# interactiveaudiolab/ppgs

Hardware: AMD Instinct MI355X
Metric: PPG frames/sec (whole node), mel repr, batch=32x1000 frames (higher is better)
Workload: dtype bf16; 1 GPU; configs[1]: mel representation, batch=32 x 1000 frames per GPU, audio resident in HBM -> (32,40,1000) fp32 posteriors in HBM; batch=32, frames=1000, per_gpu_batches=1, parallelism=utterance-sharded x1, no data-path collective

## Files before the change

### ppgs_amd/csrc/ppg_layer32.h

```cpp
#pragma once

#include "ppg_device.h"
#include "ppg_launch.h"

#include <type_traits>
#include <utility>

namespace {

constexpr float kLnEps32 = 1e-5f;
constexpr int HC = 128;

constexpr int tile_blocks(int hidt) { return hidt == 256 ? 5 : 3; }
template <int HIDT, int TBN_ = tile_blocks(HIDT)>
struct Geo {
    static_assert(HIDT == 256 || HIDT == 512, "hidden width");
    static constexpr int RB = HIDT / 128;
    static constexpr int KS = HIDT / 16;
    static constexpr int KH = KS / 16;
    static constexpr int TBN = TBN_;
    static constexpr int TOKS = 32 * TBN;
    static constexpr int HBUFS = TBN_ == tile_blocks(HIDT) ? 1 : 2;
    static constexpr int L_ACT = 0;
    static constexpr int L_H = TBN * KS * 1024;
    static constexpr int L_LNP1 = L_H + HBUFS * TBN * 8 * 1024;
    static constexpr int L_LNP2 = L_LNP1 + 3 * HIDT * 4;
    static constexpr int L_BQ = L_LNP2 + 3 * HIDT * 4;
    static constexpr int L_STATS = L_BQ + 3 * HIDT * 4;
    static constexpr int L_B1 = L_STATS + 2 * 4 * TOKS * 4;
};

__device__ __forceinline__ uint32_t lds_addr32(const void* p) {
    return (uint32_t)(uintptr_t)(const __attribute__((address_space(3))) void*)p;
}
template <int OFF>
__device__ __forceinline__ void ds_read128(u32x4& dst, uint32_t addr) {
    asm volatile("ds_read_b128 %0, %1 offset:%2" : "=v"(dst) : "v"(addr), "n"(OFF));
}
template <int N>
__device__ __forceinline__ void lgkm_wait32(u32x4& r) {
    asm volatile("s_waitcnt lgkmcnt(%1)" : "+v"(r) : "n"(N) : "memory");
    __builtin_amdgcn_sched_barrier(0);
}
template <int OFF>
__device__ __forceinline__ void gload128(u32x4& dst, uint32_t voff, const char* sbase) {
    asm volatile("global_load_dwordx4 %0, %1, %2 offset:%3" : "=v"(dst) : "v"(voff), "s"(sbase), "n"(OFF) : "memory");
}
template <int OFF>
__device__ __forceinline__ void gload128_acc(u32x4& dst, uint32_t voff, const char* sbase) {
    asm volatile("global_load_dwordx4 %0, %1, %2 offset:%3" : "=a"(dst) : "v"(voff), "s"(sbase), "n"(OFF) : "memory");
}
template <int K>
__device__ __forceinline__ void gload_frag(u32x4& dst, uint32_t voff, const char* base) {
    gload128<(K % 4) * 1024>(dst, voff, base + (K / 4) * 4096);
}
template <int K>
__device__ __forceinline__ void gload_frag_acc(u32x4& dst, uint32_t voff, const char* base) {
    gload128_acc<(K % 4) * 1024>(dst, voff, base + (K / 4) * 4096);
}
template <int COUNT>
__device__ __forceinline__ void vm_wait_all(u32x4 (&r)[COUNT]) {
    asm volatile("s_waitcnt vmcnt(0)" ::: "memory");
#pragma unroll
    for (int i = 0; i < COUNT; ++i) asm volatile("" : "+v"(r[i]));
    __builtin_amdgcn_sched_barrier(0);
}
__device__ __forceinline__ void glds16(const char* uniform_base, uint32_t lane_off, uint32_t lds_wave_addr) {
    const uint64_t b = reinterpret_cast<uint64_t>(uniform_base);
    const uint64_t base = ((uint64_t)(uint32_t)__builtin_amdgcn_readfirstlane((int)(b >> 32)) << 32) |
                          (uint64_t)(uint32_t)__builtin_amdgcn_readfirstlane((int)(uint32_t)b);
    asm volatile("s_mov_b32 m0, %2\n\ts_nop 0\n\tglobal_load_lds_dwordx4 %0, %1"
                 :: "v"(lane_off), "s"(base), "s"(__builtin_amdgcn_readfirstlane(lds_wave_addr)) : "memory", "m0");
}

template <class OFFS, int I, int N, int D, class USE>
__device__ __forceinline__ void stream_step(u32x4 (&ring)[D], uint32_t b0, uint32_t b1, USE& use) {
    if constexpr (I < N) {
        lgkm_wait32<(N - 1 - I < D - 1) ? (N - 1 - I) : (D - 1)>(ring[I % D]);
        use(std::integral_constant<int, I>{}, ring[I % D]);
        if constexpr (I + D < N) {
            constexpr int off = OFFS::at(I + D);
            if constexpr (off < 65536) ds_read128<off>(ring[I % D], b0); else ds_read128<off - 65536>(ring[I % D], b1);
        }
        stream_step<OFFS, I + 1, N, D>(ring, b0, b1, use);
    }
}
template <class OFFS, int I, int N, int D>
__device__ __forceinline__ void stream_prime(u32x4 (&ring)[D], uint32_t b0, uint32_t b1) {
    if constexpr (I < D && I < N) {
        constexpr int off = OFFS::at(I);
        if constexpr (off < 65536) ds_read128<off>(ring[I], b0); else ds_read128<off - 65536>(ring[I], b1);
        stream_prime<OFFS, I + 1, N, D>(ring, b0, b1);
    }
}
template <class OFFS, int N, int D, class USE>
__device__ __forceinline__ void stream(uint32_t b0, uint32_t b1, USE use) {
    u32x4 ring[D];
    stream_prime<OFFS, 0, N, D>(ring, b0, b1);
    stream_step<OFFS, 0, N, D>(ring, b0, b1, use);
}
template <int KS, int K0, int TB0, int NTB>
struct OffPanel { static constexpr int at(int i) { return ((TB0 + i % NTB) * KS + K0 + i / NTB) * 1024; } };
template <int TBN>
struct OffH { static constexpr int at(int i) { return ((i % TBN) * 8 + i / TBN) * 1024; } };

template <int TBN, int PAR>
struct OffH2 { static constexpr int at(int i) { return PAR * (TBN * 8 * 1024) + ((i % TBN) * 8 + i / TBN) * 1024; } };

struct OffChunk256 {
    static constexpr int at(int i) {
        constexpr int KS = Geo<256>::KS, HOFF = Geo<256>::L_H - Geo<256>::L_ACT;
        if (i < 48) return ((i % 3) * KS + i / 3) * 1024;
        if (i < 80) return ((3 + (i - 48) % 2) * KS + (i - 48) / 2) * 1024;
        if (i < 104) return HOFF + (((i - 80) % 3) * 8 + (i - 80) / 3) * 1024;
        return HOFF + ((3 + (i - 104) % 2) * 8 + (i - 104) / 2) * 1024;
    }
};

__device__ __forceinline__ void stat4(f32x2& sum2, f32x2& sq2, float v0, float v1, float v2, float v3) {
    const f32x2 a = {v0, v1}, b = {v2, v3};
    sum2 += a;
    sq2 = __builtin_elementwise_fma(a, a, sq2);
    sum2 += b;
    sq2 = __builtin_elementwise_fma(b, b, sq2);
}
__device__ __forceinline__ float hsum2(f32x2 v) {
    float r;
    asm("v_add_f32 %0, %1, %2" : "=v"(r) : "v"(v.x), "v"(v.y));
    return r;
}
__device__ __forceinline__ float pair_sum(float v) {
    auto b = __builtin_amdgcn_permlane32_swap(__float_as_uint(v), __float_as_uint(v), false, false);
    return __uint_as_float(b[0]) + __uint_as_float(b[1]);
}

template <class P, int HIDT, int TBS = tile_blocks(HIDT)>
__device__ __forceinline__ void panel_store(uint32_t pb0, int wave, int t, int rb, const f32x16& y) {
    using G = Geo<HIDT, TBS>;
#pragma unroll
    for (int s = 0; s < 2; ++s) {
        const u32x4 frag = u32x4{P::pack2(y[8 * s + 0], y[8 * s + 1]), P::pack2(y[8 * s + 2], y[8 * s + 3]),
                                 P::pack2(y[8 * s + 4], y[8 * s + 5]), P::pack2(y[8 * s + 6], y[8 * s + 7])};
        const uint32_t addr = pb0 + (uint32_t)((t * G::KS + 2 * G::RB * wave + 2 * rb + s) * 1024);
        asm volatile("ds_write_b128 %0, %1" :: "v"(addr), "v"(frag) : "memory");
    }
}

template <class P, int HIDT, int TBS = tile_blocks(HIDT)>
__device__ __forceinline__ void qkv_tail(const Layer32Args& a, char* smem, const int m0, u32x4 (&w1f)[16], u32x4 (&w2f)[16],
                                         const int nblk = TBS) {
    using G = Geo<HIDT, TBS>;
    constexpr int RB = G::RB, KS = G::KS, KH = G::KH, TB = G::TBN, TOKS = G::TOKS;
    constexpr int NSTEP = 3 * RB, NHS = NSTEP * KH;
    constexpr int NMMA = 16 * TB;
    constexpr int NU = 2 * TB;
    constexpr int USTRIDE = (NMMA - 16) / NU;
    const int lane = threadIdx.x & 63;
    const int wave = __builtin_amdgcn_readfirstlane(threadIdx.x >> 6);
    const int tok = lane & 31, hh = lane >> 5;
    const uint32_t voff = lane * 16;
    const uint32_t pb0 = lds_addr32(smem) + G::L_ACT + lane * 16, pb1 = pb0 + 65536;
    const int fbase = 32 * RB * wave;
    const f32x16 zero = {0.f, 0.f, 0.f, 0.f, 0.f, 0.f, 0.f, 0.f, 0.f, 0.f, 0.f, 0.f, 0.f, 0.f, 0.f, 0.f};
    asm volatile("s_waitcnt lgkmcnt(0)" ::: "memory");
    __syncthreads();
    const float* bq = reinterpret_cast<const float*>(smem + G::L_BQ);
    int vcol[TB][2];
    bool valigned[TB];
    bool regular = m0 + TOKS <= a.M && nblk == TB;
#pragma unroll
    for (int t = 0; t < TB; ++t) {
#pragma unroll
        for (int h = 0; h < 2; ++h) {
            const int mb = m0 + 32 * t + 16 * h;
            vcol[t][h] = -1;
            if (mb < a.M && t < nblk) {
                const int w = a.blk_win[mb >> 4];
                if (w >= 0) {
                    const int ttb = mb - a.win[w].tok_off;
                    vcol[t][h] = a.win[w].vt_off + (ttb >> 5) * 32 + 4 * ((ttb >> 4) & 1);
                }
            }
        }
        valigned[t] = vcol[t][0] >= 0 && vcol[t][1] == vcol[t][0] + 4 && (vcol[t][0] & 31) == 0;
        regular = regular && valigned[t];
    }
    const char* wq = a.wq_img + ((size_t)wave * 3 * RB * KS) * 1024;
    f32x16 acc[2][TB];
    auto bias_of = [&](auto step_tag, float4 (&b4)[4]) {
        constexpr int STEP = decltype(step_tag)::value, KIND = STEP / RB, RBI = STEP % RB;
        if constexpr (KIND < 2) {
#pragma unroll
            for (int q = 0; q < 4; ++q) b4[q] = *reinterpret_cast<const float4*>(bq + HIDT * KIND + 32 * RBI + fbase + 16 * hh + 4 * q);
        } else {
            const float bv = bq[2 * HIDT + pair_row(fbase + 32 * RBI + tok)];
            b4[0] = make_float4(bv, bv, bv, bv);
        }
    };
    auto bias_c = [&](auto step_tag) {
        constexpr int STEP = decltype(step_tag)::value;
        f32x16 cinit = zero;
        float4 bb[4];
        bias_of(step_tag, bb);
        if constexpr (STEP / RB < 2) {
#pragma unroll
            for (int q = 0; q < 4; ++q) { cinit[4 * q + 0] = bb[q].x; cinit[4 * q + 1] = bb[q].y; cinit[4 * q + 2] = bb[q].z; cinit[4 * q + 3] = bb[q].w; }
        } else {
#pragma unroll
            for (int k = 0; k < 16; ++k) cinit[k] = bb[0].x;
        }
        return cinit;
    };
    u32x4 held = u32x4{0u, 0u, 0u, 0u};
    auto unit = [&](auto step_tag, auto u_tag) {
        constexpr int STEP = decltype(step_tag)::value, U = decltype(u_tag)::value;
        constexpr int KIND = STEP / RB, RBI = STEP % RB, t = U / 2, s2 = U % 2;
        const f32x16& c = acc[STEP & 1][t];
        if (regular) {
            u32x4 r;
            if constexpr (KIND < 2) {
                r = u32x4{P::pack2(c[8 * s2 + 0], c[8 * s2 + 1]),
                          P::pack2(c[8 * s2 + 2], c[8 * s2 + 3]),
                          P::pack2(c[8 * s2 + 4], c[8 * s2 + 5]),
                          P::pack2(c[8 * s2 + 6], c[8 * s2 + 7])};
            } else {
                r = u32x4{P::pack2(c[4 * s2 + 0], c[4 * s2 + 1]), P::pack2(c[4 * s2 + 2], c[4 * s2 + 3]),
                          P::pack2(c[4 * (s2 + 2) + 0], c[4 * (s2 + 2) + 1]), P::pack2(c[4 * (s2 + 2) + 2], c[4 * (s2 + 2) + 3])};
            }
            if constexpr (s2 == 0) {
                held = r;
            } else {
                u32x4 lo, hi;
#pragma unroll
                for (int d = 0; d < 4; ++d) {
                    const auto sw = __builtin_amdgcn_permlane16_swap(held[d], r[d], false, false);
                    lo[d] = sw[0]; hi[d] = sw[1];
                }
                const int r16 = lane & 15, k16 = lane >> 4;
                if constexpr (KIND < 2) {
                    char* dst = a.qk_out + ((size_t)(m0 + 32 * t + r16) * 2 * HIDT + HIDT * KIND + 32 * RBI + fbase) * 2 + 16 * k16;
                    *reinterpret_cast<u32x4*>(dst) = lo;
                    *reinterpret_cast<u32x4*>(dst + (size_t)16 * 2 * HIDT * 2) = hi;
                } else {
                    char* dst = a.vt_out + ((size_t)(fbase + 32 * RBI + r16) * a.vt_ld + vcol[t][0]) * 2 + 16 * (2 * (k16 & 1) + (k16 >> 1));
                    *reinterpret_cast<u32x4*>(dst) = lo;
                    *reinterpret_cast<u32x4*>(dst + (size_t)16 * a.vt_ld * 2) = hi;
                }
            }
            return;
        }
        if constexpr (KIND < 2) {
            const int m = m0 + 32 * t + tok;
            if (m < a.M && t < nblk) {
                char* dst = a.qk_out + ((size_t)m * 2 * HIDT + HIDT * KIND + 32 * RBI + fbase + 16 * hh) * 2;
                *reinterpret_cast<u32x4*>(dst + 16 * s2) = u32x4{
                    P::pack2(c[8 * s2 + 0], c[8 * s2 + 1]), P::pack2(c[8 * s2 + 2], c[8 * s2 + 3]),
                    P::pack2(c[8 * s2 + 4], c[8 * s2 + 5]), P::pack2(c[8 * s2 + 6], c[8 * s2 + 7])};
            }
        } else {
            char* rowp = a.vt_out + (size_t)(fbase + 32 * RBI + tok) * a.vt_ld * 2;
            if (valigned[t]) {
                *reinterpret_cast<u32x4*>(rowp + (size_t)(vcol[t][0] + 16 * s2 + 8 * hh) * 2) = u32x4{
                    P::pack2(c[4 * s2 + 0], c[4 * s2 + 1]), P::pack2(c[4 * s2 + 2], c[4 * s2 + 3]),
                    P::pack2(c[4 * (s2 + 2) + 0], c[4 * (s2 + 2) + 1]), P::pack2(c[4 * (s2 + 2) + 2], c[4 * (s2 + 2) + 3])};
            } else if (vcol[t][s2] >= 0) {
#pragma unroll
                for (int e = 0; e < 2; ++e) {
                    const int q = 2 * s2 + e;
                    *reinterpret_cast<uint2*>(rowp + (size_t)(vcol[t][s2] + 8 * (2 * e + hh)) * 2) = make_uint2(
                        P::pack2(c[4 * q + 0], c[4 * q + 1]), P::pack2(c[4 * q + 2], c[4 * q + 3]));
                }
            }
        }
    };
    auto half_step = [&](auto hs_tag, u32x4 (&cur)[16], u32x4 (&nxt)[16]) {
        constexpr int HS = decltype(hs_tag)::value;
        constexpr int STEP = HS / KH, kh = HS % KH;
        constexpr bool SWAP = STEP / RB == 2;
        constexpr bool LAST = HS + 1 == NHS;
        constexpr bool EPI = kh == 0 && STEP > 0;
        const char* nbase = wq + (size_t)(LAST ? HS : HS + 1) * 16 * 1024;
        f32x16 cinit = zero;
        if constexpr (kh == 0) {
            cinit = bias_c(std::integral_constant<int, STEP>{});
#pragma unroll
            for (int k = 0; k < 16; ++k) asm volatile("" : "+v"(cinit[k]));
        }
        f32x16 (&c)[TB] = acc[STEP & 1];
        stream<OffPanel<KS, 16 * kh, 0, TB>, NMMA, 6>(pb0, pb1, [&](auto ic, const u32x4& bf) {
            constexpr int i = decltype(ic)::value;
            constexpr int ks = i / TB, tb = i % TB;
            if constexpr (ks == 0 && kh == 0) c[tb] = SWAP ? P::mma32(bf, cur[0], cinit) : P::mma32(cur[0], bf, cinit);
            else c[tb] = SWAP ? P::mma32(bf, cur[ks], c[tb]) : P::mma32(cur[ks], bf, c[tb]);
            if constexpr (!LAST && i < 16) gload_frag<i>(nxt[i], voff, nbase);
            if constexpr (EPI && i >= 16 && (i - 16) % USTRIDE == 0 && (i - 16) / USTRIDE < NU)
                unit(std::integral_constant<int, STEP - 1>{}, std::integral_constant<int, (i - 16) / USTRIDE>{});
        });
        if constexpr (!LAST) {
            if constexpr (EPI) {
                if (regular) asm volatile("s_waitcnt vmcnt(%0)" :: "n"(NU) : "memory");
                else asm volatile("s_waitcnt vmcnt(0)" ::: "memory");
            } else {
                asm volatile("s_waitcnt vmcnt(0)" ::: "memory");
            }
#pragma unroll
            for (int k = 0; k < 16; ++k) asm volatile("" : "+v"(nxt[k]));
            __builtin_amdgcn_sched_barrier(0);
        }
    };
    [&]<int... S>(std::integer_sequence<int, S...>) {
        ((S % 2 == 0 ? half_step(std::integral_constant<int, S>{}, w1f, w2f)
                     : half_step(std::integral_constant<int, S>{}, w2f, w1f)), ...);
    }(std::make_integer_sequence<int, NHS>{});
    (void)TOKS;
    [&]<int... U>(std::integer_sequence<int, U...>) {
        (unit(std::integral_constant<int, NSTEP - 1>{}, std::integral_constant<int, U>{}), ...);
    }(std::make_integer_sequence<int, NU>{});
}

}
```

### ppgs_amd/csrc/ppg_layer32.hip

```cpp
#include "ppg_layer32.h"

namespace {

template <class P, int HIDT, bool QKV, int TBS = tile_blocks(HIDT)>
__global__ __launch_bounds__(256) __attribute__((amdgpu_waves_per_eu(1, 1))) void layer32_kernel(Layer32Args a) {
    using G = Geo<HIDT, TBS>;
    constexpr int RB = G::RB, KS = G::KS, KH = G::KH, TB = G::TBN, TOKS = G::TOKS;
    constexpr int TBT = tile_blocks(HIDT);
    constexpr bool SUB = TBS != TBT;
    constexpr int NSUB = (TBT + TBS - 1) / TBS;
    static_assert(!SUB || (HIDT == 256 && TBS == 2), "sub-tile workgroups: hidden 256, two token blocks");
    extern __shared__ __attribute__((aligned(16))) char smem[];
    const int tid = threadIdx.x;
    const int lane = tid & 63;
    const int wave = __builtin_amdgcn_readfirstlane(tid >> 6);
    const int tok = lane & 31, hh = lane >> 5;
    const int tile = SUB ? (int)blockIdx.x / NSUB : (int)blockIdx.x;
    const int tb0 = SUB ? ((int)blockIdx.x % NSUB) * TBS : 0;
    const int nblk = SUB ? min(TBS, TBT - tb0) : TBS;
    auto gblock = [&](int t) { return SUB ? tb0 + (t < nblk ? t : -tb0) : t; };
    const int m0 = tile * (32 * TBT) + 32 * tb0;
    const int NCH = a.F / HC;
    const uint32_t lds0 = lds_addr32(smem);
    const uint32_t voff = lane * 16;
    const uint32_t pb0 = lds0 + G::L_ACT + lane * 16, pb1 = pb0 + 65536;
    const uint32_t hb0 = lds0 + G::L_H + lane * 16;
    float* lnp1 = reinterpret_cast<float*>(smem + G::L_LNP1);
    float* lnp2 = reinterpret_cast<float*>(smem + G::L_LNP2);
    float* stats = reinterpret_cast<float*>(smem + G::L_STATS);
    const int fbase = 32 * RB * wave;
    [[maybe_unused]] const char* wq_first = a.wq_img + ((size_t)wave * 3 * RB * KS) * 1024;

#ifdef PPG_FFN_TIMING
    auto pstamp = [&](int k) {
        if (a.dbg && blockIdx.x == 0 && lane == 0) a.dbg[128 + wave * 16 + k] = __builtin_amdgcn_s_memtime();
    };
#else
    auto pstamp = [&](int) {};
#endif
    pstamp(0);

    u32x4 w1f[16], w2f[16];
    auto load16 = [&](u32x4 (&wf)[16], const char* base) {
        [&]<int... K>(std::integer_sequence<int, K...>) { (gload_frag<K>(wf[K], voff, base), ...); }(std::make_integer_sequence<int, 16>{});
    };
    constexpr bool XPRE = HIDT == 256;
    constexpr int NRES = XPRE ? TB * RB * 2 : 1;
    u32x4 res[NRES];
    const bool xpre = XPRE && a.x_half;
    if (xpre) {
        const char* xbase = reinterpret_cast<const char*>(a.X) + ((size_t)tile * 4 + wave) * (TBT * RB * 2 * 1024);
        if constexpr (!SUB) {
            [&]<int... K>(std::integer_sequence<int, K...>) { (gload_frag<K>(res[K], voff, xbase), ...); }(std::make_integer_sequence<int, NRES>{});
        } else {
            [&]<int... K>(std::integer_sequence<int, K...>) {
                (gload_frag<K % (RB * 2)>(res[K], voff, xbase + (size_t)gblock(K / (RB * 2)) * (RB * 2 * 1024)), ...);
            }(std::make_integer_sequence<int, NRES>{});
        }
    }
    {
        const char* src = a.ao + (size_t)tile * (TBT * KS * 1024);
#pragma unroll
        for (int i = 0; i < TB * KS / 4; ++i) {
            const int p = 4 * i + wave;
            const int q = SUB ? gblock(p / KS) * KS + p % KS : p;
            glds16(src + (size_t)q * 1024, voff, lds0 + G::L_ACT + p * 1024);
        }
    }
    f32x16 yacc[RB][TB];
    {
        constexpr int NP = (3 * HIDT / 4 + 255) / 256;
        float4 p1[NP], p2[NP], pq[NP];
#pragma unroll
        for (int u = 0; u < NP; ++u) {
            const int i = min(tid + 256 * u, 3 * HIDT / 4 - 1);
            const int v = i / (HIDT / 4), j = i - v * (HIDT / 4);
            p1[u] = reinterpret_cast<const float4*>(v == 0 ? a.bo : (v == 1 ? a.g1 : a.e1))[j];
            p2[u] = reinterpret_cast<const float4*>(v == 0 ? a.b2 : (v == 1 ? a.g2 : a.e2))[j];
            if constexpr (QKV) pq[u] = reinterpret_cast<const float4*>(a.bq)[i];
        }
        constexpr int B1MAX = 8;
        float4 pb[B1MAX];
#pragma unroll
        for (int u = 0; u < B1MAX; ++u) pb[u] = reinterpret_cast<const float4*>(a.b1)[min(tid + 256 * u, a.F / 4 - 1)];
#pragma unroll
        for (int u = 0; u < NP; ++u) {
            const int i = tid + 256 * u;
            if (i < 3 * HIDT / 4) {
                reinterpret_cast<float4*>(lnp1)[i] = p1[u];
                reinterpret_cast<float4*>(lnp2)[i] = p2[u];
                if constexpr (QKV) reinterpret_cast<float4*>(smem + G::L_BQ)[i] = pq[u];
            }
        }
#pragma unroll
        for (int u = 0; u < B1MAX; ++u)
            if (tid + 256 * u < a.F / 4) reinterpret_cast<float4*>(smem + G::L_B1)[tid + 256 * u] = pb[u];
    }
    const f32x16 zero = {0.f, 0.f, 0.f, 0.f, 0.f, 0.f, 0.f, 0.f, 0.f, 0.f, 0.f, 0.f, 0.f, 0.f, 0.f, 0.f};
    [&]<int... R>(std::integer_sequence<int, R...>) {
        ([&] {
            constexpr int rbp = R / KH, kh = R % KH;
            const char* base = a.wo_img + ((size_t)wave * RB * KS) * 1024;
            load16(w1f, base + ((size_t)(2 * rbp) * KS + 16 * kh) * 1024);
            load16(w2f, base + ((size_t)(2 * rbp + 1) * KS + 16 * kh) * 1024);
            vm_wait_all(w1f);
            vm_wait_all(w2f);
            if constexpr (R == 0) {
#pragma unroll
                for (int k = 0; k < NRES; ++k) asm volatile("" : "+v"(res[k]));
                __syncthreads();
                pstamp(1);
            }
            if (!(PPG_DBG(a) & 1)) {
                stream<OffPanel<KS, 16 * kh, 0, TB>, 16 * TB, 6>(pb0, pb1, [&](auto ic, const u32x4& bf) {
                    constexpr int i = decltype(ic)::value;
                    constexpr int ks = i / TB, tb = i % TB;
                    if constexpr (ks == 0 && kh == 0) {
                        yacc[2 * rbp][tb] = P::mma32(w1f[0], bf, zero);
                        yacc[2 * rbp + 1][tb] = P::mma32(w2f[0], bf, zero);
                    } else {
                        yacc[2 * rbp][tb] = P::mma32(w1f[ks], bf, yacc[2 * rbp][tb]);
                        yacc[2 * rbp + 1][tb] = P::mma32(w2f[ks], bf, yacc[2 * rbp + 1][tb]);
                    }
                });
            }
        }(), ...);
    }(std::make_integer_sequence<int, (RB / 2) * KH>{});
    pstamp(2);

    float* xt = a.X + ((size_t)tile * 4 + wave) * (TBT * RB * 4 * 256) + lane * 4;
    char* xh = reinterpret_cast<char*>(a.X) + ((size_t)tile * 4 + wave) * (TBT * RB * 2 * 1024) + lane * 16;
    auto layer_norm = [&](auto residual_tag, auto xhalf_tag, const float* lnp, auto emit) {
        constexpr bool RES = decltype(residual_tag)::value;
        constexpr bool XH = decltype(xhalf_tag)::value;
        constexpr int STAMP = RES ? 7 : 9;
        constexpr bool KEEP = RB == 2;
        float4 bias4[KEEP ? RB : 1][4], gv[KEEP ? RB : 1][4], ev[KEEP ? RB : 1][4];
        auto quad = [&](int which, int rb, int q) { return *reinterpret_cast<const float4*>(lnp + which * HIDT + fbase + 32 * rb + 16 * hh + 4 * q); };
        if constexpr (KEEP) {
#pragma unroll
            for (int rb = 0; rb < RB; ++rb)
#pragma unroll
                for (int q = 0; q < 4; ++q) bias4[rb][q] = quad(0, rb, q);
        }
#pragma unroll
        for (int t = 0; t < TB; ++t) {
            f32x2 sum2 = {0.f, 0.f}, sq2 = {0.f, 0.f};
#pragma unroll
            for (int rb = 0; rb < RB; ++rb)
#pragma unroll
                for (int s2 = 0; s2 < 2; ++s2) {
                    float r8[8] = {0.f, 0.f, 0.f, 0.f, 0.f, 0.f, 0.f, 0.f};
                    [[maybe_unused]] uint32_t w4[4] = {0u, 0u, 0u, 0u};
                    if constexpr (RES && XH) {
                        u32x4 rv;
                        if constexpr (XPRE) rv = res[(t * RB + rb) * 2 + s2];
                        else rv = *reinterpret_cast<const u32x4*>(xh + ((gblock(t) * RB + rb) * 2 + s2) * 1024);
                        w4[0] = rv.x; w4[1] = rv.y; w4[2] = rv.z; w4[3] = rv.w;
                    } else if constexpr (RES) {
#pragma unroll
                        for (int e = 0; e < 2; ++e) {
                            const float4 rv = *reinterpret_cast<const float4*>(xt + ((gblock(t) * RB + rb) * 4 + 2 * s2 + e) * 256);
                            r8[4 * e + 0] = rv.x; r8[4 * e + 1] = rv.y; r8[4 * e + 2] = rv.z; r8[4 * e + 3] = rv.w;
                        }
                    }
#pragma unroll
                    for (int e = 0; e < 2; ++e) {
                        const int q = 2 * s2 + e;
                        float4 bv;
                        if constexpr (KEEP) bv = bias4[rb][q]; else bv = quad(0, rb, q);
                        if constexpr (RES && XH) {
                            const float bq4[4] = {bv.x, bv.y, bv.z, bv.w};
#pragma unroll
                            for (int k = 0; k < 4; ++k) {
                                const float sum = yacc[rb][t][4 * q + k] + bq4[k];
                                float out;
                                if (k & 1) asm("v_fma_mix_f32 %0, %1, 1.0, %2 op_sel:[1,0,0] op_sel_hi:[1,0,0]" : "=v"(out) : "v"(w4[2 * e + k / 2]), "v"(sum));
                                else asm("v_fma_mix_f32 %0, %1, 1.0, %2 op_sel:[0,0,0] op_sel_hi:[1,0,0]" : "=v"(out) : "v"(w4[2 * e + k / 2]), "v"(sum));
                                yacc[rb][t][4 * q + k] = out;
                            }
                        } else
                        {
                        yacc[rb][t][4 * q + 0] += bv.x + r8[4 * e + 0]; yacc[rb][t][4 * q + 1] += bv.y + r8[4 * e + 1];
                        yacc[rb][t][4 * q + 2] += bv.z + r8[4 * e + 2]; yacc[rb][t][4 * q + 3] += bv.w + r8[4 * e + 3];
                        }
                        stat4(sum2, sq2, yacc[rb][t][4 * q + 0], yacc[rb][t][4 * q + 1], yacc[rb][t][4 * q + 2], yacc[rb][t][4 * q + 3]);
                    }
                }
            const float sum = pair_sum(hsum2(sum2));
            const float sq = pair_sum(hsum2(sq2));
            if (hh == 0) {
                stats[wave * TOKS + 32 * t + tok] = sum;
                stats[4 * TOKS + wave * TOKS + 32 * t + tok] = sq;
            }
        }
        if constexpr (KEEP) {
#pragma unroll
            for (int rb = 0; rb < RB; ++rb)
#pragma unroll
                for (int q = 0; q < 4; ++q) { gv[rb][q] = quad(1, rb, q); ev[rb][q] = quad(2, rb, q); }
        }
        pstamp(STAMP);
        __syncthreads();
        pstamp(STAMP + 1);
#pragma unroll
        for (int t = 0; t < TB; ++t) {
            const float* s = stats + 32 * t + tok;
            const float mean = ((s[0] + s[TOKS]) + (s[2 * TOKS] + s[3 * TOKS])) * (1.0f / HIDT);
            const float ex2 = ((s[4 * TOKS] + s[5 * TOKS]) + (s[6 * TOKS] + s[7 * TOKS])) * (1.0f / HIDT);
            const float rstd = __builtin_amdgcn_rsqf(fmaxf(ex2 - mean * mean, 0.f) + kLnEps32);
            const float shift = -mean * rstd;
#pragma unroll
            for (int rb = 0; rb < RB; ++rb) {
#pragma unroll
                for (int q = 0; q < 4; ++q) {
                    float4 g4, e4;
                    if constexpr (KEEP) { g4 = gv[rb][q]; e4 = ev[rb][q]; } else { g4 = quad(1, rb, q); e4 = quad(2, rb, q); }
                    yacc[rb][t][4 * q + 0] = fmaf(fmaf(yacc[rb][t][4 * q + 0], rstd, shift), g4.x, e4.x);
                    yacc[rb][t][4 * q + 1] = fmaf(fmaf(yacc[rb][t][4 * q + 1], rstd, shift), g4.y, e4.y);
                    yacc[rb][t][4 * q + 2] = fmaf(fmaf(yacc[rb][t][4 * q + 2], rstd, shift), g4.z, e4.z);
                    yacc[rb][t][4 * q + 3] = fmaf(fmaf(yacc[rb][t][4 * q + 3], rstd, shift), g4.w, e4.w);
                }
                emit(t, rb, yacc[rb][t]);
            }
        }
    };
    auto panel_write = [&](int t, int rb, const f32x16& y) {
#pragma unroll
        for (int s = 0; s < 2; ++s) {
            const u32x4 frag = u32x4{P::pack2(y[8 * s + 0], y[8 * s + 1]), P::pack2(y[8 * s + 2], y[8 * s + 3]),
                                     P::pack2(y[8 * s + 4], y[8 * s + 5]), P::pack2(y[8 * s + 6], y[8 * s + 7])};
            const uint32_t addr = pb0 + (uint32_t)((t * KS + 2 * RB * wave + 2 * rb + s) * 1024);
            asm volatile("ds_write_b128 %0, %1" :: "v"(addr), "v"(frag) : "memory");
        }
    };
    if (a.x_half) layer_norm(std::true_type{}, std::true_type{}, lnp1, panel_write);
    else layer_norm(std::true_type{}, std::false_type{}, lnp1, panel_write);
    load16(w1f, a.w1_img + ((size_t)wave * KS) * 1024);
    asm volatile("s_waitcnt lgkmcnt(0)" ::: "memory");
    __syncthreads();
    pstamp(3);

    auto bias_read = [&](u32x4 (&braw)[4], int c) {
#pragma unroll
        for (int q = 0; q < 4; ++q) ds_read128<0>(braw[q], lds0 + G::L_B1 + (uint32_t)((c * HC + 32 * wave + 8 * q + 4 * hh) * 4));
    };
    auto bias_of = [&](u32x4 (&braw)[4]) {
        f32x16 bias;
#pragma unroll
        for (int q = 0; q < 4; ++q) {
            asm volatile("" : "+v"(braw[q]));
            bias[4 * q + 0] = __uint_as_float(braw[q].x); bias[4 * q + 1] = __uint_as_float(braw[q].y);
            bias[4 * q + 2] = __uint_as_float(braw[q].z); bias[4 * q + 3] = __uint_as_float(braw[q].w);
        }
        return bias;
    };
    if constexpr (SUB) {
        u32x4 w1g[16], w2g[16];
        f32x16 hacc[2][TB];
        u32x4 braw[4];
        auto h_write = [&](auto par_tag, auto t_tag, auto s_tag) {
            constexpr int par = decltype(par_tag)::value, t = decltype(t_tag)::value, s2 = decltype(s_tag)::value;
            const f32x16& hv = hacc[par][t];
            const u32x4 frag = u32x4{P::relu2(P::pack2(hv[8 * s2 + 0], hv[8 * s2 + 1])), P::relu2(P::pack2(hv[8 * s2 + 2], hv[8 * s2 + 3])),
                                     P::relu2(P::pack2(hv[8 * s2 + 4], hv[8 * s2 + 5])), P::relu2(P::pack2(hv[8 * s2 + 6], hv[8 * s2 + 7]))};
            const uint32_t addr = hb0 + (uint32_t)(par * (TB * 8 * 1024) + (t * 8 + 2 * wave + s2) * 1024);
            asm volatile("ds_write_b128 %0, %1" :: "v"(addr), "v"(frag) : "memory");
        };
        auto w1_of = [&](int c) { return a.w1_img + (((size_t)c * 4 + wave) * KS) * 1024; };
        auto w2_of = [&](int c) { return a.w2_img + (((size_t)c * 4 + wave) * RB * 8) * 1024; };
        const int nrun = (PPG_DBG(a) & 2) ? 0 : NCH;
        if (nrun > 0) {
            bias_read(braw, 0);
            asm volatile("s_waitcnt lgkmcnt(0)" ::: "memory");
            const f32x16 bias0 = bias_of(braw);
            vm_wait_all(w1f);
            const char* w1n = w1_of(nrun > 1 ? 1 : 0);
            const char* w20 = w2_of(0);
            stream<OffPanel<KS, 0, 0, TB>, 16 * TB, 6>(pb0, pb1, [&](auto ic, const u32x4& bf) {
                constexpr int i = decltype(ic)::value;
                constexpr int ks = i / TB, tb = i % TB;
                if constexpr (ks == 0) hacc[0][tb] = P::mma32(w1f[0], bf, bias0);
                else hacc[0][tb] = P::mma32(w1f[ks], bf, hacc[0][tb]);
                if constexpr (i < 16) gload_frag<i>(w1g[i], voff, w1n);
                else gload_frag_acc<i - 16>(w2f[i - 16], voff, w20);
                if constexpr (i == 20) bias_read(braw, nrun > 1 ? 1 : 0);
            });
        }
        auto iter = [&](auto par_tag, auto next_tag, int c) {
            constexpr int PAR = decltype(par_tag)::value;
            constexpr bool NEXT = decltype(next_tag)::value;
            u32x4 (&wa)[16] = *(PAR ? &w1f : &w1g);
            u32x4 (&wn)[16] = *(PAR ? &w1g : &w1f);
            u32x4 (&w2c)[16] = *(PAR ? &w2g : &w2f);
            u32x4 (&w2n)[16] = *(PAR ? &w2f : &w2g);
            const char* nx = c + 2 < NCH ? w1_of(c + 2) : (QKV ? wq_first : w1_of(c));
            const char* nx2 = w2_of(c + 1 < NCH ? c + 1 : c);
            const int cb = c + 2 < NCH ? c + 2 : c;
            f32x16 bias;
            if constexpr (NEXT) bias = bias_of(braw);
            asm volatile("s_waitcnt vmcnt(16)" ::: "memory");
#pragma unroll
            for (int k = 0; k < 16; ++k) asm volatile("" : "+v"(wa[k]));
            __builtin_amdgcn_sched_barrier(0);
            if constexpr (NEXT) {
                stream<OffPanel<KS, 0, 0, TB>, 16 * TB, 6>(pb0, pb1, [&](auto ic, const u32x4& bf) {
                    constexpr int i = decltype(ic)::value;
                    constexpr int ks = i / TB, tb = i % TB;
                    if constexpr (ks == 0) hacc[PAR ^ 1][tb] = P::mma32(wa[0], bf, bias);
                    else hacc[PAR ^ 1][tb] = P::mma32(wa[ks], bf, hacc[PAR ^ 1][tb]);
                    if constexpr (i % 2 == 0) gload_frag<i / 2>(wn[i / 2], voff, nx);
                    if constexpr (i % 4 == 1 && i / 4 < 2 * TB)
                        h_write(std::integral_constant<int, PAR>{}, std::integral_constant<int, (i / 4) / 2>{}, std::integral_constant<int, (i / 4) % 2>{});
                });
            } else {
                [&]<int... U>(std::integer_sequence<int, U...>) {
                    (h_write(std::integral_constant<int, PAR>{}, std::integral_constant<int, U / 2>{}, std::integral_constant<int, U % 2>{}), ...);
                }(std::make_integer_sequence<int, 2 * TB>{});
            }
            asm volatile("s_waitcnt lgkmcnt(0)" ::: "memory");
            asm volatile("s_barrier" ::: "memory");
            if constexpr (NEXT) asm volatile("s_waitcnt vmcnt(16)" ::: "memory");
            else asm volatile("s_waitcnt vmcnt(0)" ::: "memory");
#pragma unroll
            for (int k = 0; k < 16; ++k) asm volatile("" : "+a"(w2c[k]));
            __builtin_amdgcn_sched_barrier(0);
            stream<OffH2<TB, PAR>, 8 * TB, 6>(hb0, hb0, [&](auto ic, const u32x4& bf) {
                constexpr int i = decltype(ic)::value;
                constexpr int ks = i / TB, tb = i % TB;
                yacc[0][tb] = P::mma32(w2c[ks], bf, yacc[0][tb]);
                yacc[1][tb] = P::mma32(w2c[8 + ks], bf, yacc[1][tb]);
                if constexpr (NEXT) gload_frag_acc<i>(w2n[i], voff, nx2);
                if constexpr (i == 2) bias_read(braw, cb);
            });
        };
        for (int c = 0; c + 2 < nrun; c += 2) {
            iter(std::integral_constant<int, 0>{}, std::true_type{}, c);
            iter(std::integral_constant<int, 1>{}, std::true_type{}, c + 1);
        }
        if (nrun > 0) {
            iter(std::integral_constant<int, 0>{}, std::true_type{}, nrun - 2);
            iter(std::integral_constant<int, 1>{}, std::false_type{}, nrun - 1);
        }
    } else if constexpr (HIDT == 256) {
        u32x4 braw[4];
        u32x4 w2a[16];
        bias_read(braw, 0);
        asm volatile("s_waitcnt lgkmcnt(0)" ::: "memory");
        for (int c = 0; c < ((PPG_DBG(a) & 2) ? 0 : NCH); ++c) {
#ifdef PPG_FFN_TIMING
            auto cstamp = [&](int k) { if (c == 4 && a.dbg && blockIdx.x == 0 && lane == 0) a.dbg[wave * 8 + k] = __builtin_amdgcn_s_memtime(); };
#else
            auto cstamp = [&](int) {};
#endif
            cstamp(0);
            const f32x16 bias = bias_of(braw);
            vm_wait_all(w1f);
            const char* w2c = a.w2_img + (((size_t)c * 4 + wave) * RB * 8) * 1024;
            const char* next1 = c + 1 < NCH ? a.w1_img + (((size_t)(c + 1) * 4 + wave) * KS) * 1024
                                : (QKV ? wq_first : a.w1_img + (((size_t)c * 4 + wave) * KS) * 1024);
            const int cn = c + 1 < NCH ? c + 1 : c;
            f32x16 hacc[TB];
            auto h_write = [&](auto t_tag, auto s_tag) {
                constexpr int t = decltype(t_tag)::value, s2 = decltype(s_tag)::value;
                const u32x4 frag = u32x4{P::relu2(P::pack2(hacc[t][8 * s2 + 0], hacc[t][8 * s2 + 1])), P::relu2(P::pack2(hacc[t][8 * s2 + 2], hacc[t][8 * s2 + 3])),
                                         P::relu2(P::pack2(hacc[t][8 * s2 + 4], hacc[t][8 * s2 + 5])), P::relu2(P::pack2(hacc[t][8 * s2 + 6], hacc[t][8 * s2 + 7]))};
                const uint32_t addr = hb0 + (uint32_t)((t * 8 + 2 * wave + s2) * 1024);
                asm volatile("ds_write_b128 %0, %1" :: "v"(addr), "v"(frag) : "memory");
            };
            uint32_t hlo0 = 0, hlo1 = 0;
            auto h_half = [&](auto t_tag, auto s_tag, auto part_tag) {
                constexpr int t = decltype(t_tag)::value, s2 = decltype(s_tag)::value, part = decltype(part_tag)::value;
                if constexpr (part == 0) {
                    hlo0 = P::relu2(P::pack2(hacc[t][8 * s2 + 0], hacc[t][8 * s2 + 1]));
                    hlo1 = P::relu2(P::pack2(hacc[t][8 * s2 + 2], hacc[t][8 * s2 + 3]));
                } else {
                    const u32x4 frag = u32x4{hlo0, hlo1, P::relu2(P::pack2(hacc[t][8 * s2 + 4], hacc[t][8 * s2 + 5])), P::relu2(P::pack2(hacc[t][8 * s2 + 6], hacc[t][8 * s2 + 7]))};
                    const uint32_t addr = hb0 + (uint32_t)((t * 8 + 2 * wave + s2) * 1024);
                    asm volatile("ds_write_b128 %0, %1" :: "v"(addr), "v"(frag) : "memory");
                }
            };
            stream<OffChunk256, 120, 6>(pb0, pb1, [&](auto ic, const u32x4& bf) {
                constexpr int i = decltype(ic)::value;
                if constexpr (i < 48) {
                    constexpr int ks = i / 3, tb = i % 3;
                    if constexpr (ks == 0) P::mma32v0(hacc[tb], w1f[0], bf, bias);
                    else P::mma32v(hacc[tb], w1f[ks], bf);
                    if constexpr (i % 3 == 1) gload_frag_acc<i / 3>(w2a[i / 3], voff, w2c);
                } else if constexpr (i < 80) {
                    constexpr int j = i - 48, ks = j / 2, tb = 3 + j % 2;
                    if constexpr (j == 0) cstamp(1);
                    if constexpr (ks == 0) P::mma32v0(hacc[tb], w1f[0], bf, bias);
                    else P::mma32v(hacc[tb], w1f[ks], bf);
                    if constexpr (j == 4) asm volatile("" :: "v"(bias));
                    if constexpr (j >= 2 && (j - 2) % 3 < 2 && (j - 2) / 3 < 6)
                        h_half(std::integral_constant<int, ((j - 2) / 3) / 2>{}, std::integral_constant<int, ((j - 2) / 3) % 2>{}, std::integral_constant<int, (j - 2) % 3>{});
                    if constexpr (i == 74) asm volatile("s_barrier" ::: "memory");
                } else if constexpr (i < 104) {
                    constexpr int j = i - 80, ks = j / 3, tb = j % 3;
                    if constexpr (j == 0) {
                        cstamp(2);
                        asm volatile("s_waitcnt vmcnt(0)" ::: "memory");
#pragma unroll
                        for (int k = 0; k < 16; ++k) asm volatile("" : "+a"(w2a[k]));
                        __builtin_amdgcn_sched_barrier(0);
                    }
                    yacc[0][tb] = P::mma32(w2a[ks], bf, yacc[0][tb]);
                    yacc[1][tb] = P::mma32(w2a[8 + ks], bf, yacc[1][tb]);
                    if constexpr (j < 16) gload_frag<j>(w1f[j], voff, next1);
                    if constexpr (j % 3 == 1 && j / 3 < 4) h_write(std::integral_constant<int, 3 + (j / 3) / 2>{}, std::integral_constant<int, (j / 3) % 2>{});
                    if constexpr (j == 17) bias_read(braw, cn);
                    if constexpr (i == 98) asm volatile("s_barrier" ::: "memory");
                } else {
                    constexpr int j = i - 104, ks = j / 2, tb = 3 + j % 2;
                    if constexpr (j == 0) cstamp(3);
                    yacc[0][tb] = P::mma32(w2a[ks], bf, yacc[0][tb]);
                    yacc[1][tb] = P::mma32(w2a[8 + ks], bf, yacc[1][tb]);
                }
            });
            cstamp(5);
        }
    } else {
        for (int c = 0; c < ((PPG_DBG(a) & 2) ? 0 : NCH); ++c) {
#ifdef PPG_FFN_TIMING
            auto cstamp = [&](int k) { if (c == 4 && a.dbg && blockIdx.x == 0 && lane == 0) a.dbg[wave * 8 + k] = __builtin_amdgcn_s_memtime(); };
#else
            auto cstamp = [&](int) {};
#endif
            cstamp(0);
            f32x16 bias;
            {
                u32x4 braw[4];
#pragma unroll
                for (int q = 0; q < 4; ++q) ds_read128<0>(braw[q], lds0 + G::L_B1 + (uint32_t)((c * HC + 32 * wave + 8 * q + 4 * hh) * 4));
                asm volatile("s_waitcnt lgkmcnt(0)" ::: "memory");
#pragma unroll
                for (int q = 0; q < 4; ++q) {
                    asm volatile("" : "+v"(braw[q]));
                    bias[4 * q + 0] = __uint_as_float(braw[q].x); bias[4 * q + 1] = __uint_as_float(braw[q].y);
                    bias[4 * q + 2] = __uint_as_float(braw[q].z); bias[4 * q + 3] = __uint_as_float(braw[q].w);
                }
            }
            vm_wait_all(w1f);
            const char* w1c = a.w1_img + (((size_t)c * 4 + wave) * KS) * 1024;
            const char* w2c = a.w2_img + (((size_t)c * 4 + wave) * RB * 8) * 1024;
            const char* next1 = c + 1 < NCH ? a.w1_img + (((size_t)(c + 1) * 4 + wave) * KS) * 1024
                                : (QKV ? wq_first : w1c);
            f32x16 hacc[TB];
            auto h_write = [&](auto t_tag, auto s_tag) {
                constexpr int t = decltype(t_tag)::value, s2 = decltype(s_tag)::value;
                const u32x4 frag = u32x4{P::relu2(P::pack2(hacc[t][8 * s2 + 0], hacc[t][8 * s2 + 1])), P::relu2(P::pack2(hacc[t][8 * s2 + 2], hacc[t][8 * s2 + 3])),
                                         P::relu2(P::pack2(hacc[t][8 * s2 + 4], hacc[t][8 * s2 + 5])), P::relu2(P::pack2(hacc[t][8 * s2 + 6], hacc[t][8 * s2 + 7]))};
                const uint32_t addr = hb0 + (uint32_t)((t * 8 + 2 * wave + s2) * 1024);
                asm volatile("ds_write_b128 %0, %1" :: "v"(addr), "v"(frag) : "memory");
            };
                stream<OffPanel<KS, 0, 0, TB>, 16 * TB, 6>(pb0, pb1, [&](auto ic, const u32x4& bf) {
                    constexpr int i = decltype(ic)::value;
                    constexpr int ks = i / TB, tb = i % TB;
                    if constexpr (ks == 0) hacc[tb] = P::mma32(w1f[0], bf, bias);
                    else hacc[tb] = P::mma32(w1f[ks], bf, hacc[tb]);
                    if constexpr (i % 3 == 1) gload_frag<16 + i / 3>(w2f[i / 3], voff, w1c);
                });
                vm_wait_all(w2f);
                cstamp(1);
                stream<OffPanel<KS, 16, 0, TB>, 16 * TB, 6>(pb0, pb1, [&](auto ic, const u32x4& bf) {
                    constexpr int i = decltype(ic)::value;
                    constexpr int ks = i / TB, tb = i % TB;
                    if constexpr (i == 0) __builtin_amdgcn_s_barrier();
                    hacc[tb] = P::mma32(w2f[ks], bf, hacc[tb]);
                    if constexpr (i % 3 == 1) gload_frag<i / 3>(w1f[i / 3], voff, w2c);
                });
                cstamp(2);
                [&]<int... U>(std::integer_sequence<int, U...>) {
                    (h_write(std::integral_constant<int, U / 2>{}, std::integral_constant<int, U % 2>{}), ...);
                }(std::make_integer_sequence<int, 2 * TB>{});
                asm volatile("s_waitcnt lgkmcnt(0)" ::: "memory");
                cstamp(3);
                __syncthreads();
                cstamp(4);
                vm_wait_all(w1f);
                stream<OffH<TB>, 8 * TB, 6>(hb0, hb0, [&](auto ic, const u32x4& bf) {
                    constexpr int i = decltype(ic)::value;
                    constexpr int ks = i / TB, tb = i % TB;
                    yacc[0][tb] = P::mma32(w1f[ks], bf, yacc[0][tb]);
                    yacc[1][tb] = P::mma32(w1f[8 + ks], bf, yacc[1][tb]);
                    if constexpr (i < 16) gload_frag<16 + i>(w2f[i], voff, w2c);
                });
                vm_wait_all(w2f);
                stream<OffH<TB>, 8 * TB, 6>(hb0, hb0, [&](auto ic, const u32x4& bf) {
                    constexpr int i = decltype(ic)::value;
                    constexpr int ks = i / TB, tb = i % TB;
                    yacc[2][tb] = P::mma32(w2f[ks], bf, yacc[2][tb]);
                    yacc[3][tb] = P::mma32(w2f[8 + ks], bf, yacc[3][tb]);
                    if constexpr (i < 16) gload_frag<i>(w1f[i], voff, next1);
                });
            cstamp(5);
        }
    }
    vm_wait_all(w1f);
    pstamp(4);

    layer_norm(std::false_type{}, std::false_type{}, lnp2, [&](int t, int rb, const f32x16& y) {
        if (SUB && t >= nblk) {
        } else if (a.write_x && a.x_half) {
#pragma unroll
            for (int s2 = 0; s2 < 2; ++s2)
                *reinterpret_cast<u32x4*>(xh + ((gblock(t) * RB + rb) * 2 + s2) * 1024) = u32x4{pack_f16x2(y[8 * s2 + 0], y[8 * s2 + 1]), pack_f16x2(y[8 * s2 + 2], y[8 * s2 + 3]),
                                                                                  pack_f16x2(y[8 * s2 + 4], y[8 * s2 + 5]), pack_f16x2(y[8 * s2 + 6], y[8 * s2 + 7])};
        } else if (a.write_x) {
#pragma unroll
            for (int q = 0; q < 4; ++q)
                *reinterpret_cast<float4*>(xt + ((gblock(t) * RB + rb) * 4 + q) * 256) = make_float4(y[4 * q + 0], y[4 * q + 1], y[4 * q + 2], y[4 * q + 3]);
        }
        if constexpr (QKV) panel_write(t, rb, y);
        const int m = m0 + 32 * t + tok;
        if (a.Xb && m < a.M && !(SUB && t >= nblk)) {
            char* brow = a.Xb + ((size_t)m * HIDT + fbase + 32 * rb + 16 * hh) * 2;
#pragma unroll
            for (int s = 0; s < 2; ++s)
                *reinterpret_cast<u32x4*>(brow + 16 * s) = u32x4{P::pack2(y[8 * s + 0], y[8 * s + 1]), P::pack2(y[8 * s + 2], y[8 * s + 3]),
                                                                  P::pack2(y[8 * s + 4], y[8 * s + 5]), P::pack2(y[8 * s + 6], y[8 * s + 7])};
        }
    });
    pstamp(5);

    if constexpr (QKV) {
        qkv_tail<P, HIDT, TBS>(a, smem, m0, w1f, w2f, nblk);
        pstamp(6);
    }
}

template <class P, int HIDT>
hipError_t launch_layer32_h(const Layer32Args& a, hipStream_t s) {
    if (a.F % HC || a.F < HC || a.M <= 0 || a.F > 8192) return hipErrorInvalidValue;
    auto launch = [&](auto kern, auto geo, int subs) {
        using G = decltype(geo);
        const size_t lds = (size_t)G::L_B1 + (size_t)a.F * 4;
        if (lds > 163840) return hipErrorInvalidValue;
        const int tiles = (a.M + 32 * tile_blocks(HIDT) - 1) / (32 * tile_blocks(HIDT));
        static ppg::LdsLimit limit;
        const hipError_t e = limit.ensure(reinterpret_cast<const void*>(kern), lds);
        if (e != hipSuccess) return e;
        hipLaunchKernelGGL(kern, dim3(tiles * subs), dim3(256), lds, s, a);
        return hipGetLastError();
    };
    if constexpr (HIDT == 256) {
        if (a.sub_tiles) {
            if ((a.F / HC) % 2) return hipErrorInvalidValue;
            if (a.wq_img != nullptr) return launch(layer32_kernel<P, HIDT, true, 2>, Geo<HIDT, 2>{}, 3);
            return launch(layer32_kernel<P, HIDT, false, 2>, Geo<HIDT, 2>{}, 3);
        }
    }
    if (a.wq_img != nullptr) return launch(layer32_kernel<P, HIDT, true>, Geo<HIDT>{}, 1);
    return launch(layer32_kernel<P, HIDT, false>, Geo<HIDT>{}, 1);
}

template <class P>
hipError_t launch_layer32_p(const Layer32Args& a, hipStream_t s) {
    if (a.H == 256) return launch_layer32_h<P, 256>(a, s);
    if (a.H == 512) return launch_layer32_h<P, 512>(a, s);
    return hipErrorInvalidValue;
}

}

namespace ppg {

int layer32_tokens(int hidden) { return hidden == 512 ? Geo<512>::TOKS : Geo<256>::TOKS; }

int layer32_max_ffn(int hidden) { return (163840 - (hidden == 512 ? Geo<512>::L_B1 : Geo<256>::L_B1)) / 4 / HC * HC; }

hipError_t launch_layer32(int precision, const Layer32Args& a, hipStream_t s) {
    if (precision == PPG_PRECISION_BF16) return launch_layer32_p<PrecBF16>(a, s);
    if (precision == PPG_PRECISION_FP16) return launch_layer32_p<PrecF16>(a, s);
    return hipErrorInvalidValue;
}

}
```

Baseline: 48.01 million frames/s.

## Reorder layer32 prologue to overlap parameter, weight and residual loads

Restructures the kernel prologue so that the activation LDS copies, the LayerNorm/bias parameter loads (now issued as raw global_load_dwordx4), and the first output-projection weight fragments all go out before any wait. The residual prefetch is issued after them and only waited on after the first GEMM, which hides its latency behind MMA work. For hidden width 256 the second weight fragment set is loaded into AGPRs to relieve VGPR pressure. The change relies on hand-counted vmcnt values, so a mismatch could cause races, and when x_half is off the residual prefetch reads a dummy address, adding unused traffic.

```diff
diff --git a/ppgs_amd/csrc/ppg_layer32.h b/ppgs_amd/csrc/ppg_layer32.h
--- a/ppgs_amd/csrc/ppg_layer32.h
+++ b/ppgs_amd/csrc/ppg_layer32.h
@@ -57,6 +57,9 @@
 template <int K>
 __device__ __forceinline__ void gload_frag_acc(u32x4& dst, uint32_t voff, const char* base) {
     gload128_acc<(K % 4) * 1024>(dst, voff, base + (K / 4) * 4096);
+}
+__device__ __forceinline__ void gload128_lane(u32x4& dst, const void* p) {
+    asm volatile("global_load_dwordx4 %0, %1, off" : "=v"(dst) : "v"(p) : "memory");
 }
 template <int COUNT>
 __device__ __forceinline__ void vm_wait_all(u32x4 (&r)[COUNT]) {
diff --git a/ppgs_amd/csrc/ppg_layer32.hip b/ppgs_amd/csrc/ppg_layer32.hip
--- a/ppgs_amd/csrc/ppg_layer32.hip
+++ b/ppgs_amd/csrc/ppg_layer32.hip
@@ -44,12 +44,68 @@
     auto load16 = [&](u32x4 (&wf)[16], const char* base) {
         [&]<int... K>(std::integer_sequence<int, K...>) { (gload_frag<K>(wf[K], voff, base), ...); }(std::make_integer_sequence<int, 16>{});
     };
+    auto load16_acc = [&](u32x4 (&wf)[16], const char* base) {
+        [&]<int... K>(std::integer_sequence<int, K...>) { (gload_frag_acc<K>(wf[K], voff, base), ...); }(std::make_integer_sequence<int, 16>{});
+    };
     constexpr bool XPRE = HIDT == 256;
     constexpr int NRES = XPRE ? TB * RB * 2 : 1;
     u32x4 res[NRES];
     const bool xpre = XPRE && a.x_half;
-    if (xpre) {
-        const char* xbase = reinterpret_cast<const char*>(a.X) + ((size_t)tile * 4 + wave) * (TBT * RB * 2 * 1024);
+    {
+        const char* src = a.ao + (size_t)tile * (TBT * KS * 1024);
+#pragma unroll
+        for (int i = 0; i < TB * KS / 4; ++i) {
+            const int p = 4 * i + wave;
+            const int q = SUB ? gblock(p / KS) * KS + p % KS : p;
+            glds16(src + (size_t)q * 1024, voff, lds0 + G::L_ACT + p * 1024);
+        }
+    }
+    f32x16 yacc[RB][TB];
+    constexpr int NP = (3 * HIDT / 4 + 255) / 256;
+    constexpr int B1MAX = 8;
+    u32x4 p1[NP], p2[NP], pb[B1MAX];
+    [[maybe_unused]] u32x4 pq[NP];
+#pragma unroll
+    for (int u = 0; u < NP; ++u) {
+        const int i = min(tid + 256 * u, 3 * HIDT / 4 - 1);
+        const int v = i / (HIDT / 4), j = i - v * (HIDT / 4);
+        gload128_lane(p1[u], reinterpret_cast<const float4*>(v == 0 ? a.bo : (v == 1 ? a.g1 : a.e1)) + j);
+        gload128_lane(p2[u], reinterpret_cast<const float4*>(v == 0 ? a.b2 : (v == 1 ? a.g2 : a.e2)) + j);
+        if constexpr (QKV) gload128_lane(pq[u], reinterpret_cast<const float4*>(a.bq) + i);
+    }
+#pragma unroll
+    for (int u = 0; u < B1MAX; ++u) gload128_lane(pb[u], reinterpret_cast<const float4*>(a.b1) + min(tid + 256 * u, a.F / 4 - 1));
+    constexpr bool WOA = XPRE;
+    [[maybe_unused]] u32x4 woa[16];
+    u32x4 (&wo2)[16] = *(WOA ? &woa : &w2f);
+    const char* wo_base = a.wo_img + ((size_t)wave * RB * KS) * 1024;
+    load16(w1f, wo_base);
+    if constexpr (WOA) load16_acc(wo2, wo_base + (size_t)KS * 1024);
+    else load16(wo2, wo_base + (size_t)KS * 1024);
+    asm volatile("s_waitcnt vmcnt(32)" ::: "memory");
+#pragma unroll
+    for (int u = 0; u < NP; ++u) {
+        asm volatile("" : "+v"(p1[u]));
+        asm volatile("" : "+v"(p2[u]));
+        if constexpr (QKV) asm volatile("" : "+v"(pq[u]));
+    }
+#pragma unroll
+    for (int u = 0; u < B1MAX; ++u) asm volatile("" : "+v"(pb[u]));
+    __builtin_amdgcn_sched_barrier(0);
+#pragma unroll
+    for (int u = 0; u < NP; ++u) {
+        const int i = tid + 256 * u;
+        if (i < 3 * HIDT / 4) {
+            reinterpret_cast<u32x4*>(lnp1)[i] = p1[u];
+            reinterpret_cast<u32x4*>(lnp2)[i] = p2[u];
+            if constexpr (QKV) reinterpret_cast<u32x4*>(smem + G::L_BQ)[i] = pq[u];
+        }
+    }
+#pragma unroll
+    for (int u = 0; u < B1MAX; ++u)
+        if (tid + 256 * u < a.F / 4) reinterpret_cast<u32x4*>(smem + G::L_B1)[tid + 256 * u] = pb[u];
+    if constexpr (XPRE) {
+        const char* xbase = xpre ? reinterpret_cast<const char*>(a.X) + ((size_t)tile * 4 + wave) * (TBT * RB * 2 * 1024) : wo_base;
         if constexpr (!SUB) {
             [&]<int... K>(std::integer_sequence<int, K...>) { (gload_frag<K>(res[K], voff, xbase), ...); }(std::make_integer_sequence<int, NRES>{});
         } else {
@@ -57,59 +113,27 @@
                 (gload_frag<K % (RB * 2)>(res[K], voff, xbase + (size_t)gblock(K / (RB * 2)) * (RB * 2 * 1024)), ...);
             }(std::make_integer_sequence<int, NRES>{});
         }
-    }
-    {
-        const char* src = a.ao + (size_t)tile * (TBT * KS * 1024);
-#pragma unroll
-        for (int i = 0; i < TB * KS / 4; ++i) {
-            const int p = 4 * i + wave;
-            const int q = SUB ? gblock(p / KS) * KS + p % KS : p;
-            glds16(src + (size_t)q * 1024, voff, lds0 + G::L_ACT + p * 1024);
-        }
-    }
-    f32x16 yacc[RB][TB];
-    {
-        constexpr int NP = (3 * HIDT / 4 + 255) / 256;
-        float4 p1[NP], p2[NP], pq[NP];
-#pragma unroll
-        for (int u = 0; u < NP; ++u) {
-            const int i = min(tid + 256 * u, 3 * HIDT / 4 - 1);
-            const int v = i / (HIDT / 4), j = i - v * (HIDT / 4);
-            p1[u] = reinterpret_cast<const float4*>(v == 0 ? a.bo : (v == 1 ? a.g1 : a.e1))[j];
-            p2[u] = reinterpret_cast<const float4*>(v == 0 ? a.b2 : (v == 1 ? a.g2 : a.e2))[j];
-            if constexpr (QKV) pq[u] = reinterpret_cast<const float4*>(a.bq)[i];
-        }
-        constexpr int B1MAX = 8;
-        float4 pb[B1MAX];
-#pragma unroll
-        for (int u = 0; u < B1MAX; ++u) pb[u] = reinterpret_cast<const float4*>(a.b1)[min(tid + 256 * u, a.F / 4 - 1)];
-#pragma unroll
-        for (int u = 0; u < NP; ++u) {
-            const int i = tid + 256 * u;
-            if (i < 3 * HIDT / 4) {
-                reinterpret_cast<float4*>(lnp1)[i] = p1[u];
-                reinterpret_cast<float4*>(lnp2)[i] = p2[u];
-                if constexpr (QKV) reinterpret_cast<float4*>(smem + G::L_BQ)[i] = pq[u];
-            }
-        }
-#pragma unroll
-        for (int u = 0; u < B1MAX; ++u)
-            if (tid + 256 * u < a.F / 4) reinterpret_cast<float4*>(smem + G::L_B1)[tid + 256 * u] = pb[u];
-    }
+        asm volatile("s_waitcnt vmcnt(%0)" :: "n"(NRES) : "memory");
+    } else {
+        asm volatile("s_waitcnt vmcnt(0)" ::: "memory");
+    }
+#pragma unroll
+    for (int k = 0; k < 16; ++k) {
+        asm volatile("" : "+v"(w1f[k]));
+        if constexpr (WOA) asm volatile("" : "+a"(wo2[k])); else asm volatile("" : "+v"(wo2[k]));
+    }
+    __builtin_amdgcn_sched_barrier(0);
+    __syncthreads();
+    pstamp(1);
     const f32x16 zero = {0.f, 0.f, 0.f, 0.f, 0.f, 0.f, 0.f, 0.f, 0.f, 0.f, 0.f, 0.f, 0.f, 0.f, 0.f, 0.f};
     [&]<int... R>(std::integer_sequence<int, R...>) {
         ([&] {
             constexpr int rbp = R / KH, kh = R % KH;
-            const char* base = a.wo_img + ((size_t)wave * RB * KS) * 1024;
-            load16(w1f, base + ((size_t)(2 * rbp) * KS + 16 * kh) * 1024);
-            load16(w2f, base + ((size_t)(2 * rbp + 1) * KS + 16 * kh) * 1024);
-            vm_wait_all(w1f);
-            vm_wait_all(w2f);
-            if constexpr (R == 0) {
-#pragma unroll
-                for (int k = 0; k < NRES; ++k) asm volatile("" : "+v"(res[k]));
-                __syncthreads();
-                pstamp(1);
+            if constexpr (R > 0) {
+                load16(w1f, wo_base + ((size_t)(2 * rbp) * KS + 16 * kh) * 1024);
+                load16(wo2, wo_base + ((size_t)(2 * rbp + 1) * KS + 16 * kh) * 1024);
+                vm_wait_all(w1f);
+                vm_wait_all(wo2);
             }
             if (!(PPG_DBG(a) & 1)) {
                 stream<OffPanel<KS, 16 * kh, 0, TB>, 16 * TB, 6>(pb0, pb1, [&](auto ic, const u32x4& bf) {
@@ -117,16 +141,17 @@
                     constexpr int ks = i / TB, tb = i % TB;
                     if constexpr (ks == 0 && kh == 0) {
                         yacc[2 * rbp][tb] = P::mma32(w1f[0], bf, zero);
-                        yacc[2 * rbp + 1][tb] = P::mma32(w2f[0], bf, zero);
+                        yacc[2 * rbp + 1][tb] = P::mma32(wo2[0], bf, zero);
                     } else {
                         yacc[2 * rbp][tb] = P::mma32(w1f[ks], bf, yacc[2 * rbp][tb]);
-                        yacc[2 * rbp + 1][tb] = P::mma32(w2f[ks], bf, yacc[2 * rbp + 1][tb]);
+                        yacc[2 * rbp + 1][tb] = P::mma32(wo2[ks], bf, yacc[2 * rbp + 1][tb]);
                     }
                 });
             }
         }(), ...);
     }(std::make_integer_sequence<int, (RB / 2) * KH>{});
     pstamp(2);
+    if constexpr (XPRE) vm_wait_all(res);
 
     float* xt = a.X + ((size_t)tile * 4 + wave) * (TBT * RB * 4 * 256) + lane * 4;
     char* xh = reinterpret_cast<char*>(a.X) + ((size_t)tile * 4 + wave) * (TBT * RB * 2 * 1024) + lane * 16;
```

After: 48.21 million frames/s, median of 6. No clear change (+0.4%).
